# 10XGenomics/lariat

Hardware: AMD Instinct MI355X
Metric: read-pairs/sec aligned to hg38 (per-barcode align loop: SMEM seeding + SW + RFA/MAPQ on device); synthetic hg38-scale reference (higher is better)
Workload: dtype u64/i32 (FM-index + integer DP), f64 (RFA scores)

## Files before the change

include/lariat_hip.h:

```cpp
#ifndef LARIAT_HIP_H
#define LARIAT_HIP_H

#include <stddef.h>
#include <stdint.h>

#ifdef __cplusplus
extern "C" {
#endif

#define LH_ABI_VERSION 10

#define LH_OK 0
#define LH_E_ARG 1
#define LH_E_IO 2
#define LH_E_HIP 3
#define LH_E_CAPACITY 4
#define LH_E_NODEVICE 5
#define LH_E_LIMIT 6

#define LH_MAX_READ_LEN 250

typedef struct lh_index lh_index;
typedef struct lh_context lh_context;

typedef struct lh_opts {
// ... 14 lines not shown
    double improper_pair_penalty;
    double genome_length;
    int32_t run_inference;
    uint32_t flags;
} lh_opts;

#define LH_F_NO_SWEEP_FILTER 1u
#define LH_F_EXT_WAVE 16u
#define LH_F_EXT_SERIAL 32u
#define LH_F_P2_TASKS 128u
#define LH_F_RESCUE_FULL 256u
#define LH_F_SEED_LANE 512u
#define LH_F_TAIL_PASSES 1024u
#define LH_F_RFA_SLAB 2048u
#define LH_F_P2_SCAN 4096u
#define LH_F_CHAIN_WAVE 64u

typedef struct lh_index_opts {
    int32_t abi_version;
    int32_t sa_intv;
    int32_t sb_shift;
    int32_t no_kmer_table;
    int32_t no_unique_runs;
    int32_t no_sweep_filter;
    int32_t build_chunk_log2;
    int32_t ktree_levels;
} lh_index_opts;
void lh_index_opts_init(lh_index_opts* io);

typedef struct lh_context_opts {
// ... 155 lines not shown
    int32_t n_rounds;
    int32_t max_barcode;
    const int32_t* first_barcode;
    const int64_t* round_seeds;
    const int64_t* round_need_bytes;
    int64_t need_bytes;
    int64_t budget_bytes;
    int64_t max_barcode_need_bytes;
} lh_round_info;
int lh_last_rounds(lh_context* ctx, int32_t lane, lh_round_info* out);

int lh_last_rfa_classes(lh_context* ctx, int64_t* out );

int lh_last_p2_calls(lh_context* ctx, int64_t* out );

int lh_last_timings(lh_context* ctx, int32_t* n, const char* const** names, const float** ms);

int lh_stage_dump_resident(lh_context* ctx, const lh_opts* opts, lh_stage_dump** out);
void lh_stage_dump_free(lh_stage_dump* d);

int lh_get_seq(const lh_index* idx, int32_t rid, int64_t start, int64_t end, int32_t reversed, char* out );

int lh_device_memory(int device, int64_t* free_bytes, int64_t* total_bytes);
int lh_diag_random_read(int device, int64_t table_bytes, int32_t granule_bytes, int64_t n_access, double* gbps, double* ms);

int lh_diag_valu_rate(int device, int32_t op, int32_t waves_per_simd, int32_t iters, double* out, int32_t n_out);

int lh_diag_rescue_sw(int device, int32_t n_cases, const int32_t* q_off, const uint8_t* q, const int32_t* t_off, const uint8_t* t, int32_t full, int32_t weaken, int32_t* out);

int lh_diag_index_check(const lh_index* idx, uint64_t stride, uint64_t* n_checked, uint64_t* n_bad_order, uint64_t* n_bad_lf);
// ... 70 lines not shown
```

lariat_amd/capi.py:

```python
import ctypes as C
import os

import numpy as np

_HERE = os.path.dirname(os.path.abspath(__file__))
LIB_PATH = os.environ.get("LARIAT_HIP_LIB") or os.path.join(_HERE, "_build", "liblariat_hip.so")

LH_OK = 0
LH_ABI_VERSION = 10
LH_E_ARG, LH_E_IO, LH_E_HIP, LH_E_CAPACITY, LH_E_NODEVICE, LH_E_LIMIT = 1, 2, 3, 4, 5, 6
LH_REC_DEBUG_TAGS = 1
LH_F_NO_SWEEP_FILTER, LH_F_EXT_WAVE, LH_F_EXT_SERIAL, LH_F_CHAIN_WAVE, LH_F_P2_TASKS, LH_F_RESCUE_FULL, LH_F_SEED_LANE, LH_F_TAIL_PASSES, LH_F_RFA_SLAB, LH_F_P2_SCAN = 1, 16, 32, 64, 128, 256, 512, 1024, 2048, 4096
LH_MAX_READ_LEN = 250

c_i32p = C.POINTER(C.c_int32)
c_i64p = C.POINTER(C.c_int64)
c_u8p = C.POINTER(C.c_uint8)
c_u32p = C.POINTER(C.c_uint32)
c_u64p = C.POINTER(C.c_uint64)
c_f64p = C.POINTER(C.c_double)


class LhOpts(C.Structure):
    _fields_ = [
        ("abi_version", C.c_int32),
        ("a", C.c_int32), ("b", C.c_int32), ("o_del", C.c_int32), ("e_del", C.c_int32), ("o_ins", C.c_int32), ("e_ins", C.c_int32),
        ("pen_unpaired", C.c_int32), ("pen_clip5", C.c_int32), ("pen_clip3", C.c_int32),
# ... 740 lines not shown
        n = int(ri.n_rounds)
        return dict(n_rounds=n, first_barcode=_view(ri.first_barcode, n + 1 if n else 0, np.int32), round_seeds=_view(ri.round_seeds, n, np.int64),
                    round_need_bytes=_view(ri.round_need_bytes, n, np.int64), need_bytes=int(ri.need_bytes), budget_bytes=int(ri.budget_bytes),
                    max_barcode=int(ri.max_barcode), max_barcode_need_bytes=int(ri.max_barcode_need_bytes))

    def rfa_classes(self):
        out = (C.c_int64 * 4)()
        self.lib.check(self.lib.L.lh_last_rfa_classes(self.h, out))
        return dict(big=int(out[0]), rest=int(out[1]), small=int(out[2]), turned_away=int(out[3]))

    def p2_calls(self):
        out = (C.c_int64 * 4)()
        self.lib.check(self.lib.L.lh_last_p2_calls(self.h, out))
        return dict(dropped=int(out[0]), probed=int(out[1]), unprobed=int(out[2]), shares=int(out[3]))

    def stage_dump(self, batch=None, opts=None):
        opts = opts or self.lib.opts()
        if batch is not None:
            self.upload(batch)
        d = C.POINTER(LhStageDump)()
        self.lib.check(self.lib.L.lh_stage_dump_resident(self.h, C.byref(opts), C.byref(d)))
        out = StageDump(d.contents)
        self.lib.L.lh_stage_dump_free(d)
        return out


_lib = None


def load_library(path=None):
# ... 169 lines not shown
            self.h = None

    def __del__(self):
        try:
            self.close()
        except Exception:
            pass


EXPORTED_SYMBOLS = [
    "lh_last_error", "lh_device_count", "lh_opts_init", "lh_index_load", "lh_index_from_arrays", "lh_index_contigs", "lh_index_l_pac",
    "lh_index_resample_sa", "lh_index_sa_interval",
    "lh_ingest_open", "lh_ingest_next", "lh_ingest_batch_free", "lh_ingest_close", "lh_name_seed",
    "lh_records_text", "lh_records_text_ex", "lh_records_free", "lh_bam_open", "lh_bam_append", "lh_bam_set_flags", "lh_bam_close",
    "lh_index_free", "lh_index_build", "lh_context_create", "lh_context_free", "lh_align_barcodes", "lh_batch_upload", "lh_align_resident",
    "lh_result_download", "lh_result_free", "lh_last_timings", "lh_last_rounds", "lh_last_rfa_classes", "lh_last_p2_calls", "lh_stage_dump_resident", "lh_stage_dump_free", "lh_get_seq", "lh_device_memory", "lh_diag_gosort", "lh_diag_gosort_split", "lh_diag_bitonic", "lh_diag_introsort", "lh_diag_random_read", "lh_diag_valu_rate", "lh_diag_rescue_sw", "lh_diag_go_rand", "lh_diag_rescue_dedup",
    "lh_index_opts_init", "lh_context_opts_init", "lh_index_build_device", "lh_index_export", "lh_index_save", "lh_synth_genome", "lh_synth_reads", "lh_synth_write_fastq9", "lh_diag_index_check", "lh_batch_upload_slot", "lh_batch_select", "lh_bam_concat", "lh_reference_pack", "lh_index_set_holes", "lh_diag_index_digest", "lh_index_set_alt", "lh_index_alt", "lh_bam_set_level", "lh_bam_timings", "lh_result_download_begin", "lh_result_download_end", "lh_batch_stage_slot", "lh_host_alloc", "lh_host_free",
    "lh_bgzf_create", "lh_bgzf_free", "lh_bgzf_compress", "lh_bgzf_bound", "lh_bgzf_timings", "lh_bam_set_device",
    "lh_bam_set_device_records", "lh_bam_records_timings", "lh_diag_format_f6",
]
```

lariat_amd/csrc/k_smem4.h:

```cpp
#pragma once
#ifndef LH_K1_SLAB_CHUNK
#define LH_K1_SLAB_CHUNK 4
#endif
#include "lh_dev.h"
static_assert((LH_MAXLEN + 2) % LH_K1_SLAB_CHUNK == 0, "a lane's list of LH_MAXLEN + 2 entries is a whole number of chunks");
#define LH_K1_LDS_BUDGET 10240
#ifndef LH_K1_QW_SMALL
#define LH_K1_QW_SMALL 24
#endif
#ifdef LH_K1_RING
#define LH_K1_RING_OF(qw_) (LH_K1_RING)
#else
#define LH_K1_RING_OF(qw_) ((LH_K1_LDS_BUDGET - (qw_) * 256) / 2048)
#endif
static_assert(LH_K1_QW_SMALL >= 1 && LH_K1_QW_SMALL <= 32, "the small query staging holds at most the full query");

struct __attribute__((aligned(16))) PEnt { u64 lo, hi; };
#define LH_M40 0xffffffffffull
__device__ __forceinline__ PEnt pe_pack(u64 x0, u64 x1, u64 x2, int info) {
    PEnt e;
    e.lo = x0 | (x2 << 40);
    e.hi = x1 | ((x2 >> 24) << 40) | ((u64)(uint32_t)info << 49);
    return e;
}
// ... 127 lines not shown
        else { resume[r] = rs; listed = 1; }
    }
    const u64 lm = __ballot(listed);
    if (lm) {
        int basep = 0;
        if (lane == 0) basep = atomicAdd(todo_count, (int32_t)__popcll(lm));
        basep = wave_readlane(basep, 0);
        if (listed) todo[basep + lanes_below(lm, lane)] = r;
    }
    if (ctr) {
        unsigned t1 = (unsigned)wave_sum_i32((int)n_ext), t2 = (unsigned)wave_sum_i32((int)n_exec), t3 = (unsigned)wave_sum_i32((int)n_kt);
        if (lane == 0 && t1) { atomicAdd(&LH_CTR(ctr)->n_ext, (u64)t1); atomicAdd(&LH_CTR(ctr)->n_ext_exec[0], (u64)t2); atomicAdd(&LH_CTR(ctr)->n_ktree[0], (u64)t3); }
    }
}

struct K1Big { const int32_t* list; const int32_t* count; const int32_t* slot; DIntv* slab; const K1Resume* resume; };
#define LH_P2E_READ ((1ull << 27) - 1)
#define LH_P2E_SHARE (1ull << 27)
#define LH_P2E_TASK 28
#define LH_P2E_XM 28
#define LH_P2E_MIN 36
#define LH_P2E_PBITS 40
#define LH_P2E_UNPROBED (1ull << 59)
#define LH_P2_MAX_MIN_INTV 15
static_assert(LH_BLOOM_K <= 19 && LH_MAXLEN < 256, "a call entry: 8 bits of position, 19 of probe");
#define K1T_OCC 0
#define K1T_TREE 1
#define K1T_BLOOM1 2
#define K1T_BLOOM2 3
#define K1T_REPT 4
#define K1T_PLCP 5
// ... 17 lines not shown
    {                                                                                                                                            \
        if (DO12 && !BIG && lh_k1_lens) { const int v__ = (v_); atomicAdd(&lh_k1_lens[((PASS - 1) * 3 + (kind_)) * 64 + (v__ < 63 ? v__ : 63)], 1ull); } \
    }
#define K1_REQ(tab_, ptr_, bytes_)                                                                                                              \
    {                                                                                                                                            \
        if (PASS == 1 && !BIG && lh_k1_trace) {                                                                                                  \
            if (trace_k < lh_k1_trace_cap) lh_k1_trace[(size_t)trace_k * T + t] = (u64)(uintptr_t)(ptr_) | (u64)(bytes_) << 48 | (u64)(tab_) << 56; \
            ++trace_k;                                                                                                                           \
        }                                                                                                                                        \
    }
#else
#define K1_REQ(tab_, ptr_, bytes_)
#define K1_LEN(kind_, v_)
#endif

template <int PASS, bool BIG, int QW = 32>
__global__ void __launch_bounds__(64, PASS == 3 ? 8 : LH_SMEM4_WAVES) k_smem_pass(DIndex ix, DOpts o, int n_reads_all, const uint8_t* __restrict__ seq, const i64* __restrict__ seq_off,
                                               DIntv* __restrict__ intv_out, int32_t* __restrict__ n_intv, int32_t* __restrict__ status, PEnt* __restrict__ slab,
                                               int32_t* __restrict__ next_read, DCounters* __restrict__ ctr, K1Big big) {
    const int n_reads = (BIG || big.list) ? *big.count : n_reads_all;
    constexpr int ICAP = BIG ? LH_BIG_INTV : LH_MAX_INTV;
    constexpr bool DO1 = PASS == 1, DO2 = PASS == 2, DO12 = DO1 || DO2, DO3 = PASS == 3, P3T = PASS == 3;
    static_assert(QW >= 1 && QW <= 32, "query staging: 1 to 32 words per lane");
    constexpr int R = DO12 ? LH_K1_RING_OF(QW) : 0;
    static_assert(R >= 0, "ring size");
#ifndef LH_K1_RING
    static_assert(!DO12 || QW * 256 + R * 2048 <= LH_K1_LDS_BUDGET, "query + ring within the LDS of a block at LH_SMEM4_WAVES waves per SIMD");
#endif
    __shared__ uint32_t qn[(QW + 8 * R) * 64];
    const bool P2TASK = PASS == 2 && !BIG && big.list != nullptr;
// ... 187 lines not shown
#define BWD_ADVANCE()                                                                                        \
    {                                                                                                        \
        ++j;                                                                                                 \
        if (j < nprev) {                                                                                     \
            c0 = PE_X0(pn); c1 = PE_X1(pn); c2 = PE_X2(pn); cinfo = PE_INFO(pn);                             \
            st = S4_REQ_BWD;                                                                                 \
            if (j + 1 < nprev) LIST_GET((rflags & RF_REV) ? nprev - 2 - j : j, pn)                           \
        } else if (ncurr == 0) st = S4_SMEM_DONE;                                                            \
        else {                                                                                               \
            nprev = ncurr; --i;                                                                              \
            rflags = (rflags ^ RF_CURA) & ~(RF_RUNP | RF_C1UNK | RF_REV);    \
            if (i < -1) st = S4_SMEM_DONE;                                                                   \
            else { todo |= TD_ROW; st = S4_PENDING; }                                                        \
        }                                                                                                    \
    }
#define EMIT_MEM()                                                                                           \
    {                                                                                                        \
        if (cinfo - (i + 1) >= o.min_seed_len) {                                                             \
            DIntv m_; m_.x0 = c0; m_.x1 = c1; m_.x2 = c2; m_.info = (u64)(uint32_t)cinfo | (u64)(i + 1) << 32;  \
            if (P2TASK) {        \
                const int slot_ = atomicAdd(&n_intv[r], 1);                                                  \
                if (slot_ >= ICAP) ovf = 1; else out[slot_] = m_;                                            \
            } else if (on >= ICAP) ovf = 1;                                                                  \
            else { out[on] = m_; on++; K1_REQ(K1T_INTV_W, out + on - 1, 32) }                                \
        }                                                                                                    \
        last_mem_start = i + 1;                                                                              \
    }
    for (;;) {
        const bool slow_turn = __popcll(__ballot(st == S4_FETCH || (st >= 8 && st < S4_FRUN_INIT))) >= (PASS == 3 ? LH_SLOW_BATCH_P3 : PASS == 2 ? LH_SLOW_BATCH_P2 : LH_SLOW_BATCH) ||
                               !__any((st >= S4_REQ_FWD && st < 8) || st >= S4_FRUN_INIT);
        u64 need = slow_turn ? __ballot(st == S4_FETCH) : 0;
        if (need) {
            int cnt = __popcll(need), newbase = 0;
            if (chunk_next + cnt > chunk_end) {
                int nb = 0;
                if (lane == 0) nb = atomicAdd(next_read, 64);
                newbase = wave_readlane(nb, 0);
// ... 475 lines not shown
#undef K1_SLAB_IX
#undef P3_NOTEXT
#undef US0
#undef UE0
#undef US1
#undef UE1
#undef START_SMEM1
#undef WKEY_AT
#undef BLOOM_ISSUE
#undef FWD_PUSH_OK
#undef FWD_ADVANCE
#undef P3_ADVANCE
#undef BWD_ROW_BODY
#undef BWD_ADVANCE
#undef EMIT_MEM
#undef RF_RUNP
#undef RF_BT
#undef RF_C1UNK
#undef RF_PK
#undef RF_CURA
#undef RF_REV
#undef RF_TRI
#undef RF_TRIF
#undef BT_SKIP
#undef SET_BT_SKIP
#undef X_PREV
#undef SET_X_PREV
    if (ctr) {
        unsigned tot = (unsigned)wave_sum_i32((int)n_ext_total);
        if (lane == 0 && tot) atomicAdd(&LH_CTR(ctr)->n_ext, (u64)tot);
// ... 188 lines not shown
    for (int u = 0; u < n; ++u) {
        DIntv p = a[u];
        if (p.x2 <= (u64)o.max_occ) continue;
        int sb = (int)(p.info >> 32), se = (int)(uint32_t)p.info;
        if (sb > e) { l_rep += e - b; b = sb; e = se; }
        else e = e > se ? e : se;
    }
    return l_rep + e - b;
}
__device__ __forceinline__ int dev_seed_count(const DOpts& o, u64 s) {
    if (s <= (u64)o.max_occ) return (int)s;
    u64 step = s / (u64)o.max_occ;
    u64 c = (s + step - 1) / step;
    return (int)(c < (u64)o.max_occ ? c : (u64)o.max_occ);
}
#define LH_CNT_REP 0x1000000u
#define LH_CNT_OVF 0x80000000u
__device__ __forceinline__ uint32_t dev_cnt_acc(const DOpts& o, u64 s) { return s > (u64)o.max_occ || s >= LH_CNT_REP ? LH_CNT_REP : (uint32_t)s; }
__global__ void __launch_bounds__(256) k_smem_p3_lock(DIndex ix, DOpts o, int n_reads, const uint32_t* __restrict__ q4, const i64* __restrict__ seq_off, DIntv* __restrict__ intv_out,
                                                       int32_t* __restrict__ n_intv, int32_t* __restrict__ status, DCounters* __restrict__ ctr,
                                                       int32_t* __restrict__ seed_cnt, int32_t* __restrict__ l_rep, int32_t* __restrict__ fin_list, int32_t* __restrict__ fin_count) {
    const int r = blockIdx.x * blockDim.x + threadIdx.x, lane = LANE();
    const PEnt* const kt = (const PEnt*)ix.ktree;
    const int ktl = kt ? ix.ktree_levels : 0;
    const int Lw = o.min_seed_len + 1;
    const bool text_ok = ix.isa != nullptr && ix.plcp != nullptr && o.max_mem_intv > 1;
    unsigned n_ext = 0, n_exec = 0, n_kt = 0;
    uint32_t cnt = 0;
    int fin = 0;
    if (r < n_reads) {
        const i64 off = seq_off[r];
        int len = (int)(seq_off[r + 1] - off);
        int on = n_intv[r];
// ... 92 lines not shown
            fin = on > 16 || (cnt & ~LH_CNT_OVF) >= LH_CNT_REP;
        }
    }
    if (seed_cnt) {
        const u64 m = __ballot(fin);
        int base = 0;
        if (lane == 0 && m) base = atomicAdd(fin_count, __popcll(m));
        base = wave_readlane(base, 0);
        if (fin) fin_list[base + lanes_below(m, lane)] = r;
    }
    if (ctr) {
        unsigned t1 = (unsigned)wave_sum_i32((int)n_ext), t2 = (unsigned)wave_sum_i32((int)n_exec), t3 = (unsigned)wave_sum_i32((int)n_kt);
        if (lane == 0 && t1) { atomicAdd(&LH_CTR(ctr)->n_ext, (u64)t1); atomicAdd(&LH_CTR(ctr)->n_ext_exec[2], (u64)t2); atomicAdd(&LH_CTR(ctr)->n_ktree[2], (u64)t3); }
    }
}

#define LH_FIN_GRID 4096
__global__ void __launch_bounds__(256) k_smem_fin(DOpts o, int n_reads, DIntv* __restrict__ intv, const int32_t* __restrict__ n_intv, int32_t* __restrict__ seed_cnt,
                                                   int32_t* __restrict__ l_rep_out, const int32_t* __restrict__ big_slot, const int32_t* __restrict__ list,
                                                   const int32_t* __restrict__ list_count) {
    const int n_items = list ? *list_count : n_reads, sub = threadIdx.x & 15;
    for (int g0 = blockIdx.x * (blockDim.x >> 4); g0 < n_items; g0 += gridDim.x * (blockDim.x >> 4)) {
        const int gid = g0 + (threadIdx.x >> 4);
        const int item = gid < n_items ? gid : n_items - 1;
        const int r = list ? list[item] : item;
        const int live = gid < n_items && !(big_slot && big_slot[r] >= 0);
        DIntv* a = intv + (size_t)r * LH_MAX_INTV;
        const int n = live ? n_intv[r] : 0;
        DIntv mine[4];
        int rank[4];
// ... 80 lines not shown
```

lariat_amd/csrc/lh_host.inc:

```
#include <math.h>
#include <stdlib.h>
#include <stdio.h>
#include <string.h>

#include <algorithm>
#include <array>
#include <functional>
#include <memory>
#include <mutex>
#include <string>
#include <vector>
#include <deque>
#include <map>

#include "../../include/lariat_hip.h"
#include "k_smem4.h"
#include "k_chain_lane.h"
#include "k_chain_cl.h"
#include "k_rfa.h"
#include "k_rescue3.h"
#include "k_rounds.h"
#include "lh_result_cols.h"

static void lh_print_wd(const int32_t* d_wd) {
// ... 481 lines not shown
        K1Big first = nobig; first.list = c->d_k1_todo; first.count = &c->d_next_read->n_todo; first.resume = c->d_k1_resume;
        const int g3 = (N + 63) / 64 < 2 * c->grid_smem4 ? (N + 63) / 64 : 2 * c->grid_smem4;
        T_BEGIN("k_smem4");
        LH_LAUNCH(k_smem_first, (N + 255) / 256, 256, c->stream, ix4, o, N, q4, (const i64*)c->b.seq_off, c->d_intv, c->d_n_intv, c->d_status, c->d_k1_resume, c->d_k1_todo, &c->d_next_read->n_todo, c->d_ctr);
#ifdef LH_K1_TRACE
        K1Trace trace;
        { int rc = k1_trace_begin(c, trace, g4); if (rc) return rc; }
#endif
        const bool qw_small = c->b.max_len <= 8 * LH_K1_QW_SMALL;
        if (qw_small) smem_pass<1, false, LH_K1_QW_SMALL>(c, ix4, o, N, g4, first);
        else smem_pass<1, false>(c, ix4, o, N, g4, first);
        T_END();
#ifdef LH_K1_TRACE
        { int rc = k1_trace_replay(c, trace, N, g4); if (rc) return rc; }
#endif
        T_BEGIN("k_smem4_p2");
        HIPCHK(hipMemsetAsync(c->d_p2_calls, 0, sizeof(P2Calls) * LH_CTR_SLOTS, c->stream));
        const bool p2_list_ok = N < (1 << 27);
        bool p2_probe = p2_list_ok && !(c->flags & (LH_F_P2_TASKS | LH_F_P2_SCAN)) && o.split_width < LH_P2_MAX_MIN_INTV;
#ifdef LH_K1_TRACE
        p2_probe = false;
#endif
        const bool p2_tasks = p2_list_ok && !p2_probe && ((c->flags & LH_F_P2_TASKS) || (c->ext_hint_valid && c->h_peek->prev_wave_reads >= ext_long_min(N)));
        K1Big p2 = nobig;
        if (p2_probe || p2_tasks) { p2.list = (const int32_t*)c->d_p2_tasks; p2.count = &c->d_next_read->n_p2_tasks; p2.slot = c->d_k1_todo; }
        if (p2_probe)
            LH_LAUNCH(k_p2_probe, (N + 255) / 256, 256, c->stream, ix4, o, N, (const uint8_t*)c->b.seq, (const i64*)c->b.seq_off, (const DIntv*)c->d_intv, (const int32_t*)c->d_n_intv, c->d_p2_tasks,
                      &c->d_next_read->n_p2_tasks, c->d_k1_todo, c->d_p2_calls);
        else if (p2_tasks)
            LH_LAUNCH(k_p2_tasks, (N + 255) / 256, 256, c->stream, o, N, (const DIntv*)c->d_intv, (const int32_t*)c->d_n_intv, c->d_p2_tasks, &c->d_next_read->n_p2_tasks, c->d_k1_todo, c->d_p2_calls);
        if (qw_small) smem_pass<2, false, LH_K1_QW_SMALL>(c, ix4, o, N, g4, p2);
        else smem_pass<2, false>(c, ix4, o, N, g4, p2);
        if (p2_probe || p2_tasks) LH_LAUNCH(k_p2_clamp, (N + 255) / 256, 256, c->stream, N, c->d_n_intv);
        T_END();
#ifdef LH_K1_TRACE
        { int rc = k1_trace_lens(c, trace); if (rc) return rc; }
#endif
        T_BEGIN("k_smem4_p3");
        bool p3_counts = o.max_mem_intv > 0 && q4 && !(c->flags & LH_F_SEED_LANE);
#ifdef LH_K1_TRACE
        p3_counts = false;
#endif
        if (o.max_mem_intv > 0 && q4)
            LH_LAUNCH(k_smem_p3_lock, (N + 255) / 256, 256, c->stream, ix4, o, N, q4, (const i64*)c->b.seq_off, c->d_intv, c->d_n_intv, c->d_status, c->d_ctr,
                      p3_counts ? c->d_seed_cnt : nullptr, p3_counts ? c->d_l_rep : nullptr, p3_counts ? c->d_fin_list : nullptr, p3_counts ? &c->d_next_read->n_fin : nullptr);
        else if (o.max_mem_intv > 0)
            smem_pass<3, false>(c, ix4, o, N, g3, nobig);
        T_END();
        T_BEGIN("k_smem_fin");
        { int rc = k1_big_round(c, o, ix4, N, 0); if (rc) return rc; }
        { int rc = smem_fin(c, o, N, p3_counts); if (rc) return rc; }
        T_END();
    }
    T_BEGIN("k_scan_seeds");
    { int rc = run_scan(c, N, c->d_seed_cnt, 0, 0, c->d_seed_off, c->d_reg_off, LH_RESCUE_SLOTS); if (rc) return rc; }
    T_END();
    {
        { int rc = peek_seed_total(c, N); if (rc) return rc; }
        while (c->h_peek->k1.big_asked > (i64)(c->big_cap - c->big_base)) {
            const i64 asked = c->h_peek->k1.big_asked, old_cap = c->big_cap, new_cap = old_cap + asked + asked / 8 + 16;
            if (new_cap > (1 << 30)) return set_err(LH_E_CAPACITY, "too many reads with more than LH_MAX_INTV SMEM intervals for one batch: split the batch");
            DIntv* slab = nullptr; int32_t* list = nullptr;
            DevGroup grown;
// ... 221 lines not shown
            if (acc) lh_result_free(acc);
            return set_err(rc, why);
        }
    }
    c->round_result = acc;
    R.n_rounds = (int)n_rounds;
    c->n_t = sums.n;
    for (int i = 0; i < sums.n; ++i) { c->tnames[i] = sums.names[i]; c->tms[i] = sums.ms[i]; }
    return LH_OK;
}

static int pipe_align(lh_context* c, const lh_opts* opts) {
    if (!c || !opts) return set_err(LH_E_ARG, "lh_align_resident: null argument");
    if (!c->resident) return set_err(LH_E_ARG, "no batch resident: call lh_batch_upload first");
    if (opts->abi_version != LH_ABI_VERSION) return set_err(LH_E_ARG, "lh_opts.abi_version does not match LH_ABI_VERSION (use lh_opts_init)");
    if (opts->flags & ~(LH_F_NO_SWEEP_FILTER | LH_F_EXT_WAVE | LH_F_EXT_SERIAL | LH_F_CHAIN_WAVE | LH_F_P2_TASKS | LH_F_RESCUE_FULL | LH_F_SEED_LANE | LH_F_TAIL_PASSES | LH_F_RFA_SLAB | LH_F_P2_SCAN)) return set_err(LH_E_ARG, "lh_opts.flags: unknown bit set");
    HIPCHK(hipSetDevice(c->idx->device));
    {
        std::vector<void*> fl;
        { std::lock_guard<std::mutex> g(c->slot_mu); fl.swap(c->free_later); }
        for (void* q : fl) hipFree(q);
    }
    if (c->round_result) { lh_result_free(c->round_result); c->round_result = nullptr; }
    c->rounds.clear();
    c->ran = false;
    if (!c->pool_cap) { int rc = alloc_seed_pools(c, first_pool_cap(c)); if (rc) return rc; }
    if (!c->cand_cap) { int rc = alloc_cand_pools(c, first_cand_cap(c)); if (rc) return rc; }
    DOpts o = to_dopts(opts);
    o.wd = c->d_wd;
    c->flags = opts->flags;
    int t = 0;
// ... 121 lines not shown
```

lariat_amd/csrc/lh_lanes.inc:

```
#include <atomic>
#include <thread>

#define LH_MAX_LANES 4

int lh_context_create(lh_index* idx, int64_t max_pairs, const lh_context_opts* co, lh_context** out) {
    const int lanes = co && co->lanes ? co->lanes : 1;
    if (lanes < 1 || lanes > LH_MAX_LANES) return set_err(LH_E_ARG, "lh_context_opts.lanes must be 1 .. 4");
    lh_context* c = nullptr;
    int rc = pipe_create(idx, max_pairs, co, &c);
    if (rc) return rc;
    for (int k = 1; k < lanes && max_pairs >= 2 * lanes; ++k) {
        lh_context_opts c2 = *co;
        c2.lanes = 1;
        {
            const int g = (c2.rfa_grid > 0 ? c2.rfa_grid : 4096) / lanes;
            c2.rfa_grid = g > 1024 ? g : 1024;
        }
        int64_t cap = max_pairs / lanes + 30000 < max_pairs ? max_pairs / lanes + 30000 : max_pairs;
        lh_context* p = nullptr;
        rc = pipe_create(idx, cap, &c2, &p);
        if (rc) { lh_context_free(c); return rc; }
        c->more.push_back(p);
    }
    *out = c;
// ... 130 lines not shown
}

int lh_last_rfa_classes(lh_context* c, int64_t* out) {
    if (!c || !out) return set_err(LH_E_ARG, "lh_last_rfa_classes: null argument");
    if (!c->ran_inference) return set_err(LH_E_ARG, "lh_last_rfa_classes: call lh_align_resident with run_inference first");
    for (int i = 0; i < 4; ++i) out[i] = c->rfa_cls[i];
    return LH_OK;
}

int lh_last_p2_calls(lh_context* c, int64_t* out) {
    if (!c || !out) return set_err(LH_E_ARG, "lh_last_p2_calls: null argument");
    for (int i = 0; i < 4; ++i) out[i] = c->p2_cls[i];
    return LH_OK;
}

static int merge_into(lh_result*& acc, lh_result* part) {
    if (!acc) { acc = part; return LH_OK; }
    lh_result* m = nullptr;
    const int rc = merge_results(acc, part, &m);
    lh_result_free(acc); lh_result_free(part);
    acc = m;
    return rc;
}
static int merge_results(lh_result* a, lh_result* b, lh_result** out) {
    const size_t Ca = (size_t)a->n_cand, Cb = (size_t)b->n_cand;
    size_t total = 0;
    auto reserve = [&](size_t bytes) { size_t o = total; total += (bytes + 63) & ~(size_t)63; return o; };
    std::array<size_t, LH_N_COLS> na, nb, off;
    for (size_t i = 0; i < LH_N_COLS; ++i) {
        const ResultCol& k = LH_RESULT_COLS[i];
// ... 113 lines not shown
```

Before: 54.81 million.

## Fuse SMEM pass-2 probe with pass-3 lock and reorder p3 before p2

Adds a fused k_p23_lock kernel that performs the pass-2 bloom probe and task emission together with the pass-3 text-locked reseeding in one launch over reads. It runs before the pass-2 split tasks, and a new k_p2_close kernel finalizes seed counts and the fin list. Pass-2 emits now add their counts atomically into seed_cnt. The goal is to save one full sweep over each read's intervals, plus a launch and an extra read of the interval array. The cost is an atomic per pass-2 seed and a different order of seed emission. The old order stays available behind a new LH_F_P3_LAST flag, and a fin_list query API is added for checking.

```diff
diff --git a/include/lariat_hip.h b/include/lariat_hip.h
--- a/include/lariat_hip.h
+++ b/include/lariat_hip.h
@@ -8,7 +8,7 @@
 extern "C" {
 #endif
 
-#define LH_ABI_VERSION 10
+#define LH_ABI_VERSION 11
 
 #define LH_OK 0
 #define LH_E_ARG 1
@@ -53,6 +53,7 @@
 #define LH_F_TAIL_PASSES 1024u
 #define LH_F_RFA_SLAB 2048u
 #define LH_F_P2_SCAN 4096u
+#define LH_F_P3_LAST 8192u
 #define LH_F_CHAIN_WAVE 64u
 
 typedef struct lh_index_opts {
@@ -238,6 +239,8 @@
 
 int lh_last_p2_calls(lh_context* ctx, int64_t* out );
 
+int lh_last_fin_list(lh_context* ctx, int32_t* out, int64_t cap, int64_t* n);
+
 int lh_last_timings(lh_context* ctx, int32_t* n, const char* const** names, const float** ms);
 
 int lh_stage_dump_resident(lh_context* ctx, const lh_opts* opts, lh_stage_dump** out);
diff --git a/lariat_amd/capi.py b/lariat_amd/capi.py
--- a/lariat_amd/capi.py
+++ b/lariat_amd/capi.py
@@ -7,10 +7,10 @@
 LIB_PATH = os.environ.get("LARIAT_HIP_LIB") or os.path.join(_HERE, "_build", "liblariat_hip.so")
 
 LH_OK = 0
-LH_ABI_VERSION = 10
+LH_ABI_VERSION = 11
 LH_E_ARG, LH_E_IO, LH_E_HIP, LH_E_CAPACITY, LH_E_NODEVICE, LH_E_LIMIT = 1, 2, 3, 4, 5, 6
 LH_REC_DEBUG_TAGS = 1
-LH_F_NO_SWEEP_FILTER, LH_F_EXT_WAVE, LH_F_EXT_SERIAL, LH_F_CHAIN_WAVE, LH_F_P2_TASKS, LH_F_RESCUE_FULL, LH_F_SEED_LANE, LH_F_TAIL_PASSES, LH_F_RFA_SLAB, LH_F_P2_SCAN = 1, 16, 32, 64, 128, 256, 512, 1024, 2048, 4096
+LH_F_NO_SWEEP_FILTER, LH_F_EXT_WAVE, LH_F_EXT_SERIAL, LH_F_CHAIN_WAVE, LH_F_P2_TASKS, LH_F_RESCUE_FULL, LH_F_SEED_LANE, LH_F_TAIL_PASSES, LH_F_RFA_SLAB, LH_F_P2_SCAN, LH_F_P3_LAST = 1, 16, 32, 64, 128, 256, 512, 1024, 2048, 4096, 8192
 LH_MAX_READ_LEN = 250
 
 c_i32p = C.POINTER(C.c_int32)
@@ -781,6 +781,15 @@
         self.lib.check(self.lib.L.lh_last_p2_calls(self.h, out))
         return dict(dropped=int(out[0]), probed=int(out[1]), unprobed=int(out[2]), shares=int(out[3]))
 
+    def fin_list(self):
+        L = self.lib.L
+        L.lh_last_fin_list.argtypes = [C.c_void_p, c_i32p, C.c_int64, C.POINTER(C.c_int64)]
+        n = C.c_int64()
+        self.lib.check(L.lh_last_fin_list(self.h, None, 0, C.byref(n)))
+        out = np.zeros(max(int(n.value), 1), dtype=np.int32)
+        self.lib.check(L.lh_last_fin_list(self.h, out.ctypes.data_as(c_i32p), len(out), C.byref(n)))
+        return np.sort(out[:int(n.value)])
+
     def stage_dump(self, batch=None, opts=None):
         opts = opts or self.lib.opts()
         if batch is not None:
@@ -980,7 +989,7 @@
     "lh_ingest_open", "lh_ingest_next", "lh_ingest_batch_free", "lh_ingest_close", "lh_name_seed",
     "lh_records_text", "lh_records_text_ex", "lh_records_free", "lh_bam_open", "lh_bam_append", "lh_bam_set_flags", "lh_bam_close",
     "lh_index_free", "lh_index_build", "lh_context_create", "lh_context_free", "lh_align_barcodes", "lh_batch_upload", "lh_align_resident",
-    "lh_result_download", "lh_result_free", "lh_last_timings", "lh_last_rounds", "lh_last_rfa_classes", "lh_last_p2_calls", "lh_stage_dump_resident", "lh_stage_dump_free", "lh_get_seq", "lh_device_memory", "lh_diag_gosort", "lh_diag_gosort_split", "lh_diag_bitonic", "lh_diag_introsort", "lh_diag_random_read", "lh_diag_valu_rate", "lh_diag_rescue_sw", "lh_diag_go_rand", "lh_diag_rescue_dedup",
+    "lh_result_download", "lh_result_free", "lh_last_timings", "lh_last_rounds", "lh_last_rfa_classes", "lh_last_p2_calls", "lh_last_fin_list", "lh_stage_dump_resident", "lh_stage_dump_free", "lh_get_seq", "lh_device_memory", "lh_diag_gosort", "lh_diag_gosort_split", "lh_diag_bitonic", "lh_diag_introsort", "lh_diag_random_read", "lh_diag_valu_rate", "lh_diag_rescue_sw", "lh_diag_go_rand", "lh_diag_rescue_dedup",
     "lh_index_opts_init", "lh_context_opts_init", "lh_index_build_device", "lh_index_export", "lh_index_save", "lh_synth_genome", "lh_synth_reads", "lh_synth_write_fastq9", "lh_diag_index_check", "lh_batch_upload_slot", "lh_batch_select", "lh_bam_concat", "lh_reference_pack", "lh_index_set_holes", "lh_diag_index_digest", "lh_index_set_alt", "lh_index_alt", "lh_bam_set_level", "lh_bam_timings", "lh_result_download_begin", "lh_result_download_end", "lh_batch_stage_slot", "lh_host_alloc", "lh_host_free",
     "lh_bgzf_create", "lh_bgzf_free", "lh_bgzf_compress", "lh_bgzf_bound", "lh_bgzf_timings", "lh_bam_set_device",
     "lh_bam_set_device_records", "lh_bam_records_timings", "lh_diag_format_f6",
diff --git a/lariat_amd/csrc/k_smem4.h b/lariat_amd/csrc/k_smem4.h
--- a/lariat_amd/csrc/k_smem4.h
+++ b/lariat_amd/csrc/k_smem4.h
@@ -165,7 +165,7 @@
     }
 }
 
-struct K1Big { const int32_t* list; const int32_t* count; const int32_t* slot; DIntv* slab; const K1Resume* resume; };
+struct K1Big { const int32_t* list; const int32_t* count; const int32_t* slot; DIntv* slab; union { const K1Resume* resume; int32_t* p2_cnt; }; };
 #define LH_P2E_READ ((1ull << 27) - 1)
 #define LH_P2E_SHARE (1ull << 27)
 #define LH_P2E_TASK 28
@@ -213,6 +213,10 @@
 #define K1_LEN(kind_, v_)
 #endif
 
+#define LH_CNT_REP 0x1000000u
+#define LH_CNT_OVF 0x80000000u
+__device__ __forceinline__ uint32_t dev_cnt_acc(const DOpts& o, u64 s) { return s > (u64)o.max_occ || s >= LH_CNT_REP ? LH_CNT_REP : (uint32_t)s; }
+static_assert((unsigned long long)LH_MAX_INTV * LH_CNT_REP < LH_CNT_OVF, "a read's count word: LH_MAX_INTV adds of at most LH_CNT_REP stay below the overflow bit");
 template <int PASS, bool BIG, int QW = 32>
 __global__ void __launch_bounds__(64, PASS == 3 ? 8 : LH_SMEM4_WAVES) k_smem_pass(DIndex ix, DOpts o, int n_reads_all, const uint8_t* __restrict__ seq, const i64* __restrict__ seq_off,
                                                DIntv* __restrict__ intv_out, int32_t* __restrict__ n_intv, int32_t* __restrict__ status, PEnt* __restrict__ slab,
@@ -430,13 +434,19 @@
             else { todo |= TD_ROW; st = S4_PENDING; }                                                        \
         }                                                                                                    \
     }
+#ifdef LH_P23_NO_P2_COUNT
+#define P2_COUNT_ADD()
+#else
+#define P2_COUNT_ADD() { if (big.p2_cnt) atomicAdd(&big.p2_cnt[r], (int)dev_cnt_acc(o, c2)); }
+#endif
 #define EMIT_MEM()                                                                                           \
     {                                                                                                        \
         if (cinfo - (i + 1) >= o.min_seed_len) {                                                             \
             DIntv m_; m_.x0 = c0; m_.x1 = c1; m_.x2 = c2; m_.info = (u64)(uint32_t)cinfo | (u64)(i + 1) << 32;  \
             if (P2TASK) {        \
                 const int slot_ = atomicAdd(&n_intv[r], 1);                                                  \
-                if (slot_ >= ICAP) ovf = 1; else out[slot_] = m_;                                            \
+                if (slot_ >= ICAP) ovf = 1;                                                                  \
+                else { out[slot_] = m_; P2_COUNT_ADD() }                                                     \
             } else if (on >= ICAP) ovf = 1;                                                                  \
             else { out[on] = m_; on++; K1_REQ(K1T_INTV_W, out + on - 1, 32) }                                \
         }                                                                                                    \
@@ -942,6 +952,7 @@
 #undef BWD_ROW_BODY
 #undef BWD_ADVANCE
 #undef EMIT_MEM
+#undef P2_COUNT_ADD
 #undef RF_RUNP
 #undef RF_BT
 #undef RF_C1UNK
@@ -1160,9 +1171,6 @@
     u64 c = (s + step - 1) / step;
     return (int)(c < (u64)o.max_occ ? c : (u64)o.max_occ);
 }
-#define LH_CNT_REP 0x1000000u
-#define LH_CNT_OVF 0x80000000u
-__device__ __forceinline__ uint32_t dev_cnt_acc(const DOpts& o, u64 s) { return s > (u64)o.max_occ || s >= LH_CNT_REP ? LH_CNT_REP : (uint32_t)s; }
 __global__ void __launch_bounds__(256) k_smem_p3_lock(DIndex ix, DOpts o, int n_reads, const uint32_t* __restrict__ q4, const i64* __restrict__ seq_off, DIntv* __restrict__ intv_out,
                                                        int32_t* __restrict__ n_intv, int32_t* __restrict__ status, DCounters* __restrict__ ctr,
                                                        int32_t* __restrict__ seed_cnt, int32_t* __restrict__ l_rep, int32_t* __restrict__ fin_list, int32_t* __restrict__ fin_count) {
@@ -1285,6 +1293,256 @@
         if (lane == 0 && t1) { atomicAdd(&LH_CTR(ctr)->n_ext, (u64)t1); atomicAdd(&LH_CTR(ctr)->n_ext_exec[2], (u64)t2); atomicAdd(&LH_CTR(ctr)->n_ktree[2], (u64)t3); }
     }
 }
+#ifdef LH_P3_KINDS
+__device__ unsigned long long lh_p3_kinds[16];
+#define P3K_DECL() unsigned k3_[16] = {0, 0, 0, 0, 0, 0, 0, 0, 0, 0, 0, 0, 0, 0, 0, 0}; int kk_ = 0; unsigned ke_ = 0, kt_ = 0;
+#define P3K_ADD(i_, v_) k3_[i_] += (unsigned)(v_);
+#define P3K_BEGIN()                                                                                                          \
+    {                                                                                                                        \
+        kk_ = 1; ke_ = n_exec; kt_ = n_kt;                                                                                   \
+        for (int k_ = 0; k_ < (int)n_pass1[r]; ++k_) {                                                                       \
+            const DIntv p_ = out[k_];                                                                                        \
+            const int ps_ = (int)(p_.info >> 32), pe_ = (int)(uint32_t)p_.info;                                              \
+            if (p_.x2 == 1 && !in0 && !in1 && x >= ps_ && x + Lw <= pe_) kk_ = 0;                                            \
+        }                                                                                                                    \
+        if (x + o.min_seed_len >= len) kk_ = 2;                                                                              \
+    }
+#define P3K_END() { k3_[5 + kk_] += 1; k3_[8 + kk_] += n_exec - ke_; k3_[11 + kk_] += n_kt - kt_; }
+#define P3K_FLUSH()                                                                                                          \
+    for (int i_ = 0; i_ < 14; ++i_) { const unsigned t_ = (unsigned)wave_sum_i32((int)k3_[i_]); if (lane == 0 && t_) atomicAdd(&lh_p3_kinds[i_], (unsigned long long)t_); }
+#else
+#define P3K_DECL()
+#define P3K_ADD(i_, v_)
+#define P3K_BEGIN()
+#define P3K_END()
+#define P3K_FLUSH()
+#endif
+__global__ void __launch_bounds__(256, 6) k_p23_lock(DIndex ix, DOpts o, int n_reads, const uint8_t* __restrict__ seq, const uint32_t* __restrict__ q4, const i64* __restrict__ seq_off,
+                                                   DIntv* __restrict__ intv_out, int32_t* __restrict__ n_intv, DCounters* __restrict__ ctr, int32_t* __restrict__ seed_cnt,
+                                                   u64* __restrict__ tasks, int32_t* __restrict__ n_tasks, int32_t* __restrict__ n_pass1, P2Calls* __restrict__ calls) {
+    __shared__ u64 ent[LH_P2_SPLIT * 256];
+    const int r = blockIdx.x * blockDim.x + threadIdx.x, lane = LANE();
+    const bool probe = ix.bloom1 != nullptr && ix.rep_t != nullptr && o.min_seed_len >= LH_BLOOM_K;
+    const int split_len = (int)(o.min_seed_len * o.split_factor + .499);
+#ifdef LH_P2_PROBE_WEAK
+    const u64 pmask = (1ull << (LH_BLOOM_K - 1)) - 1;
+#else
+    const u64 pmask = (1ull << LH_BLOOM_K) - 1;
+#endif
+    const int Lw = o.min_seed_len + 1;
+    const bool text_ok = ix.isa != nullptr && ix.plcp != nullptr && o.max_mem_intv > 1;
+    int m = 0, n_drop = 0, n_prob = 0, n_unpr = 0, share = 0;
+    i64 off = 0;
+    int len = 0, on = 0;
+    uint32_t uspan = 0, cnt = 0;
+    u64 up0 = 0, up1 = 0;
+    if (r < n_reads) {
+        off = seq_off[r];
+        len = (int)(seq_off[r + 1] - off);
+        if (len > LH_MAXLEN || len < o.min_seed_len || o.max_mem_intv <= 0) len = 0;
+        on = n_intv[r] < LH_MAX_INTV ? n_intv[r] : LH_MAX_INTV;
+        n_pass1[r] = on;
+        const bool pick = text_ok && len > 0;
+        const uint4* const iv = (const uint4*)(intv_out + (size_t)r * LH_MAX_INTV);
+        for (int k0 = 0; k0 < on; k0 += 4) {
+            uint2 lo[4];
+            uint4 hi[4];
+#pragma unroll
+            for (int q = 0; q < 4; ++q) {
+                lo[q] = uint2{0, 0}; hi[q] = uint4{0, 0, 0, 0};
+                if (k0 + q < on) { lo[q] = *(const uint2*)&iv[2 * (k0 + q)]; hi[q] = iv[2 * (k0 + q) + 1]; }
+            }
+#pragma unroll
+            for (int q = 0; q < 4; ++q) {
+                if (k0 + q >= on) continue;
+                const int ps = (int)hi[q].w, pe = (int)hi[q].z;
+                const u64 x0 = (u64)lo[q].x | (u64)lo[q].y << 32, x2 = (u64)hi[q].x | (u64)hi[q].y << 32;
+                cnt += dev_cnt_acc(o, x2);
+                if (!pick || x2 != 1 || pe - ps < Lw) continue;
+                const int l0 = (int)((uspan >> 8) & 0xff) - (int)(uspan & 0xff), l1 = (int)(uspan >> 24) - (int)((uspan >> 16) & 0xff);
+                const uint32_t sp = (uint32_t)ps | (uint32_t)pe << 8;
+                if (pe - ps > l0) { uspan = uspan << 16 | sp; up1 = up0; up0 = x0; }
+                else if (pe - ps > l1) { uspan = (uspan & 0xffffu) | sp << 16; up1 = x0; }
+            }
+            const bool last = k0 + 4 >= on;
+            u64 s0 = up0 & ~LH_POSF, s1 = up1 & ~LH_POSF;
+            const bool rd0 = last && (uspan & 0xffffu) && !(up0 & LH_POSF), rd1 = last && (uspan >> 16) && !(up1 & LH_POSF);
+            if (rd0) s0 = ix.sa[up0];
+            if (rd1) s1 = ix.sa[up1];
+            bool call[4], in[4];
+            int xm[4], w0[4];
+            uint32_t base[4];
+            u64 pos[4];
+#pragma unroll
+            for (int q = 0; q < 4; ++q) {
+                const int s = (int)hi[q].w, e = (int)hi[q].z;
+                const u64 x0 = (u64)lo[q].x | (u64)lo[q].y << 32, x2 = (u64)hi[q].x | (u64)hi[q].y << 32;
+                call[q] = k0 + q < on && e - s >= split_len && x2 <= (u64)o.split_width;
+                xm[q] = (s + e) >> 1; w0[q] = xm[q] - (LH_BLOOM_K - 1) - s;
+                in[q] = call[q] && probe && w0[q] >= 0 && xm[q] + LH_BLOOM_K <= e;
+                base[q] = 4; pos[q] = x0 & ~LH_POSF;
+                if (call[q]) base[q] = seq[off + xm[q]];
+                if (in[q] && !(x0 & LH_POSF)) pos[q] = ix.sa[x0];
+            }
+            u64 b0[4], b1[4];
+#pragma unroll
+            for (int q = 0; q < 4; ++q) {
+                call[q] = call[q] && base[q] <= 3;
+                in[q] = in[q] && call[q];
+                b0[q] = b1[q] = 0; pos[q] += (u64)w0[q];
+                if (in[q]) { b0[q] = ix.rep_t[pos[q] >> 6]; b1[q] = ix.rep_t[(pos[q] >> 6) + 1]; }
+            }
+            if (last) { up0 = s0; up1 = s1; }
+#pragma unroll
+            for (int q = 0; q < 4; ++q) {
+                if (!call[q]) continue;
+                const uint32_t sh = (uint32_t)(pos[q] & 63);
+                const u64 pbits = (sh ? (b0[q] >> sh) | (b1[q] << (64 - sh)) : b0[q]) & pmask;
+                if (in[q] && !pbits) { ++n_drop; continue; }
+                if (in[q]) ++n_prob; else ++n_unpr;
+                const u64 min_intv = ((u64)hi[q].x | (u64)hi[q].y << 32) + 1;
+                if (m < LH_P2_SPLIT)
+                    ent[m * 256 + threadIdx.x] = (u64)(uint32_t)r | (u64)xm[q] << LH_P2E_XM | min_intv << LH_P2E_MIN | (in[q] ? pbits << LH_P2E_PBITS : LH_P2E_UNPROBED);
+                ++m;
+            }
+        }
+        if (m > LH_P2_SPLIT) { share = 1; m = LH_P2_SPLIT; n_prob = n_unpr = 0; }
+    }
+    {
+        const int incl = wave_scan_add_i32(m);
+        const int tot = wave_readlane(incl, 63);
+        int basep = 0;
+        if (lane == 0 && tot) basep = atomicAdd(n_tasks, tot);
+        basep = wave_readlane(basep, 0);
+        for (int j = 0; j < m; ++j) tasks[basep + incl - m + j] = share ? p2_share_entry(r, j, m) : ent[j * 256 + threadIdx.x];
+        const int t_drop = wave_sum_i32(n_drop), t_prob = wave_sum_i32(n_prob), t_unpr = wave_sum_i32(n_unpr), t_sh = __popcll(__ballot(share));
+        if (lane == 0) {
+            if (t_drop) atomicAdd(&LH_CTR(calls)->dropped, (u64)t_drop);
+            if (t_prob) atomicAdd(&LH_CTR(calls)->probed, (u64)t_prob);
+            if (t_unpr) atomicAdd(&LH_CTR(calls)->unprobed, (u64)t_unpr);
+            if (t_sh) atomicAdd(&LH_CTR(calls)->shares, (u64)t_sh);
+        }
+    }
+    const PEnt* const kt = (const PEnt*)ix.ktree;
+    const int ktl = kt ? ix.ktree_levels : 0;
+    unsigned n_ext = 0, n_exec = 0, n_kt = 0;
+    P3K_DECL()
+    if (r < n_reads) {
+        DIntv* out = intv_out + (size_t)r * LH_MAX_INTV;
+#define QN(i_) ((int)(dev_nib8(q4, off + (i_)) & 0xf))
+#define P23_US0 ((int)(uspan & 0xff))
+#define P23_UE0 ((int)((uspan >> 8) & 0xff))
+#define P23_US1 ((int)((uspan >> 16) & 0xff))
+#define P23_UE1 ((int)(uspan >> 24))
+        int x = 0, notext = 0;
+        P3K_ADD(0, 1) P3K_ADD(1, on)
+        while (x < len) {
+            if (QN(x) > 3) { ++x; continue; }
+            const int in0 = x >= P23_US0 && x + Lw <= P23_UE0, in1 = x >= P23_US1 && x + Lw <= P23_UE1;
+            if (text_ok && !notext && (in0 || in1)) {
+                const i64 tp = in0 ? (i64)up0 + (x - P23_US0) : (i64)up1 + (x - P23_US1);
+                if ((int)ix.plcp[tp] < Lw) {
+                    if (on >= LH_MAX_INTV) cnt |= LH_CNT_OVF;
+                    else {
+                        DIntv mm; mm.x0 = LH_POSF | (u64)tp; mm.x1 = 0; mm.x2 = 1; mm.info = (u64)x << 32 | (u64)(x + Lw); out[on++] = mm;
+                        cnt += dev_cnt_acc(o, 1);
+                    }
+                    n_ext += (unsigned)(Lw - 1);
+                    x += Lw;
+                    P3K_ADD(4, 1)
+                    continue;
+                }
+                notext = 1;
+            }
+            notext = 0;
+            P3K_BEGIN()
+            DIntv c = dev_set_intv(ix, QN(x));
+            int i = x + 1;
+            uint32_t fcode = (uint32_t)QN(x);
+            if (ktl > 1 && x + ktl <= len && o.min_seed_len >= ktl) {
+                uint32_t w0 = dev_nib8(q4, off + x), w1 = dev_nib8(q4, off + x + 8);
+                uint32_t m0 = w0, m1 = w1;
+                if (ktl < 8) { m0 &= (1u << (4 * ktl)) - 1u; m1 = 0; }
+                else if (ktl < 16) m1 &= (1u << (4 * (ktl - 8))) - 1u;
+                if (!((m0 | m1) & 0x44444444u)) {
+                    uint32_t ca = w0 & 0x33333333u, cb = w1 & 0x33333333u;
+                    ca = (ca | ca >> 2) & 0x0f0f0f0fu; ca = (ca | ca >> 4) & 0x00ff00ffu; ca = (ca | ca >> 8) & 0xffffu;
+                    cb = (cb | cb >> 2) & 0x0f0f0f0fu; cb = (cb | cb >> 4) & 0x00ff00ffu; cb = (cb | cb >> 8) & 0xffffu;
+                    const uint32_t code = (ca | cb << 16) & (ktl >= 16 ? 0xffffffffu : (1u << (2 * ktl)) - 1u);
+                    const PEnt te = kt[(((1ull << (2 * ktl)) - 4) / 3) + code];
+                    c.x0 = PE_X0(te); c.x1 = PE_X1(te); c.x2 = PE_X2(te);
+                    n_ext += (unsigned)(ktl - 1);
+                    i = x + ktl;
+                }
+            }
+            int nx = len;
+            for (; i < len; ++i) {
+                const int b = QN(i);
+                if (b > 3) { nx = i + 1; break; }
+                DIntv ok;
+                const int lnew = i + 1 - x;
+                if (lnew <= ktl) {
+                    fcode |= (uint32_t)b << (2 * (lnew - 1));
+                    const PEnt te = kt[(((1ull << (2 * lnew)) - 4) / 3) + fcode];
+                    ok.x0 = PE_X0(te); ok.x1 = PE_X1(te); ok.x2 = PE_X2(te); ok.info = 0;
+                    ++n_kt;
+                } else { ok = dev_extend_c(ix, c, 3 - b, 0); ++n_exec; }
+                ++n_ext;
+                if (ok.x2 < (u64)o.max_mem_intv && i - x >= o.min_seed_len) {
+                    if (ok.x2 > 0) {
+                        if (on >= LH_MAX_INTV) cnt |= LH_CNT_OVF;
+                        else {
+                            ok.info = (u64)x << 32 | (u64)(i + 1); out[on++] = ok;
+                            cnt += dev_cnt_acc(o, ok.x2);
+                        }
+                    }
+                    nx = i + 1;
+                    break;
+                }
+                c = ok;
+            }
+            x = nx;
+            P3K_END()
+        }
+#undef QN
+#undef P23_US0
+#undef P23_UE0
+#undef P23_US1
+#undef P23_UE1
+        P3K_ADD(2, on - n_pass1[r])
+        n_intv[r] = on;
+        seed_cnt[r] = (int)cnt;
+    }
+    P3K_FLUSH()
+    if (ctr) {
+        unsigned t1 = (unsigned)wave_sum_i32((int)n_ext), t2 = (unsigned)wave_sum_i32((int)n_exec), t3 = (unsigned)wave_sum_i32((int)n_kt);
+        if (lane == 0 && t1) { atomicAdd(&LH_CTR(ctr)->n_ext, (u64)t1); atomicAdd(&LH_CTR(ctr)->n_ext_exec[2], (u64)t2); atomicAdd(&LH_CTR(ctr)->n_ktree[2], (u64)t3); }
+    }
+}
+__global__ void __launch_bounds__(256) k_p2_close(int n_reads, int32_t* __restrict__ n_intv, int32_t* __restrict__ status, int32_t* __restrict__ seed_cnt, int32_t* __restrict__ l_rep,
+                                                   int32_t* __restrict__ fin_list, int32_t* __restrict__ fin_count) {
+    const int r = blockIdx.x * blockDim.x + threadIdx.x, lane = LANE();
+    int fin = 0;
+    if (r < n_reads) {
+        int on = n_intv[r];
+        if (on > LH_MAX_INTV) n_intv[r] = on = LH_MAX_INTV;
+        const uint32_t cnt = (uint32_t)seed_cnt[r];
+        if (cnt & LH_CNT_OVF) status[r] |= LH_ST_INTV_OVERFLOW;
+        seed_cnt[r] = (int)(cnt & (LH_CNT_REP - 1)); l_rep[r] = 0;
+        fin = on > 16 || (cnt & ~LH_CNT_OVF) >= LH_CNT_REP;
+#ifdef LH_P3_KINDS
+        atomicAdd(&lh_p3_kinds[3], (unsigned long long)on);
+#endif
+    }
+#ifdef LH_P23_NO_FIN_LIST
+    fin = 0;
+#endif
+    const u64 m = __ballot(fin);
+    int base = 0;
+    if (lane == 0 && m) base = atomicAdd(fin_count, __popcll(m));
+    base = wave_readlane(base, 0);
+    if (fin) fin_list[base + lanes_below(m, lane)] = r;
+}
 
 #define LH_FIN_GRID 4096
 __global__ void __launch_bounds__(256) k_smem_fin(DOpts o, int n_reads, DIntv* __restrict__ intv, const int32_t* __restrict__ n_intv, int32_t* __restrict__ seed_cnt,
diff --git a/lariat_amd/csrc/lh_host.inc b/lariat_amd/csrc/lh_host.inc
--- a/lariat_amd/csrc/lh_host.inc
+++ b/lariat_amd/csrc/lh_host.inc
@@ -519,7 +519,6 @@
 #ifdef LH_K1_TRACE
         { int rc = k1_trace_replay(c, trace, N, g4); if (rc) return rc; }
 #endif
-        T_BEGIN("k_smem4_p2");
         HIPCHK(hipMemsetAsync(c->d_p2_calls, 0, sizeof(P2Calls) * LH_CTR_SLOTS, c->stream));
         const bool p2_list_ok = N < (1 << 27);
         bool p2_probe = p2_list_ok && !(c->flags & (LH_F_P2_TASKS | LH_F_P2_SCAN)) && o.split_width < LH_P2_MAX_MIN_INTV;
@@ -527,31 +526,58 @@
         p2_probe = false;
 #endif
         const bool p2_tasks = p2_list_ok && !p2_probe && ((c->flags & LH_F_P2_TASKS) || (c->ext_hint_valid && c->h_peek->prev_wave_reads >= ext_long_min(N)));
-        K1Big p2 = nobig;
-        if (p2_probe || p2_tasks) { p2.list = (const int32_t*)c->d_p2_tasks; p2.count = &c->d_next_read->n_p2_tasks; p2.slot = c->d_k1_todo; }
-        if (p2_probe)
-            LH_LAUNCH(k_p2_probe, (N + 255) / 256, 256, c->stream, ix4, o, N, (const uint8_t*)c->b.seq, (const i64*)c->b.seq_off, (const DIntv*)c->d_intv, (const int32_t*)c->d_n_intv, c->d_p2_tasks,
-                      &c->d_next_read->n_p2_tasks, c->d_k1_todo, c->d_p2_calls);
-        else if (p2_tasks)
-            LH_LAUNCH(k_p2_tasks, (N + 255) / 256, 256, c->stream, o, N, (const DIntv*)c->d_intv, (const int32_t*)c->d_n_intv, c->d_p2_tasks, &c->d_next_read->n_p2_tasks, c->d_k1_todo, c->d_p2_calls);
-        if (qw_small) smem_pass<2, false, LH_K1_QW_SMALL>(c, ix4, o, N, g4, p2);
-        else smem_pass<2, false>(c, ix4, o, N, g4, p2);
-        if (p2_probe || p2_tasks) LH_LAUNCH(k_p2_clamp, (N + 255) / 256, 256, c->stream, N, c->d_n_intv);
-        T_END();
-#ifdef LH_K1_TRACE
-        { int rc = k1_trace_lens(c, trace); if (rc) return rc; }
-#endif
-        T_BEGIN("k_smem4_p3");
-        bool p3_counts = o.max_mem_intv > 0 && q4 && !(c->flags & LH_F_SEED_LANE);
+        const bool p3_lock = o.max_mem_intv > 0 && q4;
+        bool p3_counts = p3_lock && !(c->flags & LH_F_SEED_LANE);
 #ifdef LH_K1_TRACE
         p3_counts = false;
 #endif
-        if (o.max_mem_intv > 0 && q4)
-            LH_LAUNCH(k_smem_p3_lock, (N + 255) / 256, 256, c->stream, ix4, o, N, q4, (const i64*)c->b.seq_off, c->d_intv, c->d_n_intv, c->d_status, c->d_ctr,
-                      p3_counts ? c->d_seed_cnt : nullptr, p3_counts ? c->d_l_rep : nullptr, p3_counts ? c->d_fin_list : nullptr, p3_counts ? &c->d_next_read->n_fin : nullptr);
-        else if (o.max_mem_intv > 0)
-            smem_pass<3, false>(c, ix4, o, N, g3, nobig);
-        T_END();
+        const bool p23 = p2_probe && p3_counts && !(c->flags & LH_F_P3_LAST);
+        K1Big p2 = nobig;
+        if (p2_probe || p2_tasks) { p2.list = (const int32_t*)c->d_p2_tasks; p2.count = &c->d_next_read->n_p2_tasks; p2.slot = c->d_k1_todo; }
+        if (p23) {
+            T_BEGIN("k_smem4_p3");
+            LH_LAUNCH(k_p23_lock, (N + 255) / 256, 256, c->stream, ix4, o, N, (const uint8_t*)c->b.seq, q4, (const i64*)c->b.seq_off, c->d_intv, c->d_n_intv, c->d_ctr, c->d_seed_cnt, c->d_p2_tasks,
+                      &c->d_next_read->n_p2_tasks, c->d_k1_todo, c->d_p2_calls);
+            T_END();
+            T_BEGIN("k_smem4_p2");
+            p2.p2_cnt = c->d_seed_cnt;
+            if (qw_small) smem_pass<2, false, LH_K1_QW_SMALL>(c, ix4, o, N, g4, p2);
+            else smem_pass<2, false>(c, ix4, o, N, g4, p2);
+            LH_LAUNCH(k_p2_close, (N + 255) / 256, 256, c->stream, N, c->d_n_intv, c->d_status, c->d_seed_cnt, c->d_l_rep, c->d_fin_list, &c->d_next_read->n_fin);
+            T_END();
+#ifdef LH_P3_KINDS
+            {
+                unsigned long long k[16], zero[16] = {0};
+                HIPCHK(hipStreamSynchronize(c->stream));
+                HIPCHK(hipMemcpyFromSymbol(k, HIP_SYMBOL(lh_p3_kinds), sizeof k));
+                HIPCHK(hipMemcpyToSymbol(HIP_SYMBOL(lh_p3_kinds), zero, sizeof zero));
+                fprintf(stderr, "[lh] p3_kinds:");
+                for (int i = 0; i < 14; ++i) fprintf(stderr, " %llu", k[i]);
+                fprintf(stderr, "\n");
+            }
+#endif
+        } else {
+            T_BEGIN("k_smem4_p2");
+            if (p2_probe)
+                LH_LAUNCH(k_p2_probe, (N + 255) / 256, 256, c->stream, ix4, o, N, (const uint8_t*)c->b.seq, (const i64*)c->b.seq_off, (const DIntv*)c->d_intv, (const int32_t*)c->d_n_intv, c->d_p2_tasks,
+                          &c->d_next_read->n_p2_tasks, c->d_k1_todo, c->d_p2_calls);
+            else if (p2_tasks)
+                LH_LAUNCH(k_p2_tasks, (N + 255) / 256, 256, c->stream, o, N, (const DIntv*)c->d_intv, (const int32_t*)c->d_n_intv, c->d_p2_tasks, &c->d_next_read->n_p2_tasks, c->d_k1_todo, c->d_p2_calls);
+            if (qw_small) smem_pass<2, false, LH_K1_QW_SMALL>(c, ix4, o, N, g4, p2);
+            else smem_pass<2, false>(c, ix4, o, N, g4, p2);
+            if (p2_probe || p2_tasks) LH_LAUNCH(k_p2_clamp, (N + 255) / 256, 256, c->stream, N, c->d_n_intv);
+            T_END();
+#ifdef LH_K1_TRACE
+            { int rc = k1_trace_lens(c, trace); if (rc) return rc; }
+#endif
+            T_BEGIN("k_smem4_p3");
+            if (p3_lock)
+                LH_LAUNCH(k_smem_p3_lock, (N + 255) / 256, 256, c->stream, ix4, o, N, q4, (const i64*)c->b.seq_off, c->d_intv, c->d_n_intv, c->d_status, c->d_ctr,
+                          p3_counts ? c->d_seed_cnt : nullptr, p3_counts ? c->d_l_rep : nullptr, p3_counts ? c->d_fin_list : nullptr, p3_counts ? &c->d_next_read->n_fin : nullptr);
+            else if (o.max_mem_intv > 0)
+                smem_pass<3, false>(c, ix4, o, N, g3, nobig);
+            T_END();
+        }
         T_BEGIN("k_smem_fin");
         { int rc = k1_big_round(c, o, ix4, N, 0); if (rc) return rc; }
         { int rc = smem_fin(c, o, N, p3_counts); if (rc) return rc; }
@@ -803,7 +829,7 @@
     if (!c || !opts) return set_err(LH_E_ARG, "lh_align_resident: null argument");
     if (!c->resident) return set_err(LH_E_ARG, "no batch resident: call lh_batch_upload first");
     if (opts->abi_version != LH_ABI_VERSION) return set_err(LH_E_ARG, "lh_opts.abi_version does not match LH_ABI_VERSION (use lh_opts_init)");
-    if (opts->flags & ~(LH_F_NO_SWEEP_FILTER | LH_F_EXT_WAVE | LH_F_EXT_SERIAL | LH_F_CHAIN_WAVE | LH_F_P2_TASKS | LH_F_RESCUE_FULL | LH_F_SEED_LANE | LH_F_TAIL_PASSES | LH_F_RFA_SLAB | LH_F_P2_SCAN)) return set_err(LH_E_ARG, "lh_opts.flags: unknown bit set");
+    if (opts->flags & ~(LH_F_NO_SWEEP_FILTER | LH_F_EXT_WAVE | LH_F_EXT_SERIAL | LH_F_CHAIN_WAVE | LH_F_P2_TASKS | LH_F_RESCUE_FULL | LH_F_SEED_LANE | LH_F_TAIL_PASSES | LH_F_RFA_SLAB | LH_F_P2_SCAN | LH_F_P3_LAST)) return set_err(LH_E_ARG, "lh_opts.flags: unknown bit set");
     HIPCHK(hipSetDevice(c->idx->device));
     {
         std::vector<void*> fl;
diff --git a/lariat_amd/csrc/lh_lanes.inc b/lariat_amd/csrc/lh_lanes.inc
--- a/lariat_amd/csrc/lh_lanes.inc
+++ b/lariat_amd/csrc/lh_lanes.inc
@@ -168,6 +168,19 @@
     return LH_OK;
 }
 
+int lh_last_fin_list(lh_context* c, int32_t* out, int64_t cap, int64_t* n) {
+    if (!c || !n || cap < 0 || (cap && !out)) return set_err(LH_E_ARG, "lh_last_fin_list: null argument");
+    if (!c->d_fin_list || !c->d_next_read) return set_err(LH_E_ARG, "lh_last_fin_list: call lh_align_resident or lh_stage_dump_resident first");
+    HIPCHK(hipSetDevice(c->idx->device));
+    HIPCHK(hipStreamSynchronize(c->stream));
+    int32_t n_fin = 0;
+    HIPCHK(hipMemcpy(&n_fin, &c->d_next_read->n_fin, sizeof n_fin, hipMemcpyDeviceToHost));
+    *n = n_fin;
+    const int64_t k = n_fin < cap ? n_fin : cap;
+    if (k > 0) HIPCHK(hipMemcpy(out, c->d_fin_list, (size_t)k * sizeof(int32_t), hipMemcpyDeviceToHost));
+    return LH_OK;
+}
+
 static int merge_into(lh_result*& acc, lh_result* part) {
     if (!acc) { acc = part; return LH_OK; }
     lh_result* m = nullptr;
```

Result: faster. 55.55 million (median of 6 runs) (+1.3%).
